# openfheorg/openfhe-development

Hardware: AMD Instinct MI355X
Metric: NTT GB/s vs HBM roofline + CKKS EvalMultKeySwitch/sec, N=2^16 L=30, 1/2/4/8 GPU (higher is better)
Workload: dtype u64; 1 GPU; batched fwd+inv negacyclic NTT, N=2^16, L=30 x 60-bit limbs, 1024 polynomials per GPU (BASELINE configs[1]); global_batch=1024, parallelism=batch-sharded x1, no data-path collective

## Files before the change

openfhe-development_amd/csrc/basis_kernels.h:

```cpp
#ifndef FHE_BASIS_KERNELS_H
#define FHE_BASIS_KERNELS_H
#include "modarith.h"
#include "launch.h"
#include "ntt_kernels.h"
#include "elemwise_kernels.h"
#include "ntt_static.h"

namespace fhe {


struct ConvTables {
    const TwPair* hatInv;
    const uint64_t* hatMod;
    const uint64_t* srcQ;
    const uint64_t* dstQ;
    const uint64_t* dstMu;
    const uint64_t* dstRed;
    const double* srcQInv;
    const uint64_t* alphaMod;
};

struct ConvArgs {
    const uint64_t* in;
    uint64_t* out;
// ... 48 lines not shown
        for (uint32_t i = 0; i < g.nSrcAll; ++i) {
            const uint64_t yi = mul_shoup(ina[(uint64_t)i << g.logN], hpa[2 * i], hpa[2 * i + 1], g.allSrcQ[i]);
            nu += (double)yi * g.allQInv[i];
        }
    }
    const uint32_t alpha = EXACT && (!CHUNK || g.last) ? (uint32_t)nu : 0u;

    for (uint32_t j = 0; j < g.nDst; ++j) {
        uint64_t h[NSRC];
#pragma unroll
        for (int i = 0; i < NSRC; ++i)
            h[i] = FHE_ULOAD64(g.tb.hatMod, (uint64_t)j * NSRC + i);
        const uint64_t p = FHE_ULOAD64(g.tb.dstQ, j);
        const uint64_t mulo = FHE_ULOAD64(g.tb.dstMu, 2 * j), muhi = FHE_ULOAD64(g.tb.dstMu, 2 * j + 1);
        if (SUM8 == 2) {
            const uint32_t k = 64u - (uint32_t)__builtin_clzll(p);
            uint64_t v       = 0;
#pragma unroll
            for (int c0 = 0; c0 < NSRC; c0 += 8) {
                if (c0 && c0 >= (int)g.nSrc)
                    break;
                sum8s s8;
                sum8s_clear(s8);
#pragma unroll
                for (int i = c0; i < c0 + 8 && i < NSRC; ++i) {
                    uint32_t y0, y1, h0, h1;
                    split30(y[i], y0, y1);
                    split30(h[i], h0, h1);
                    sum8s_add(s8, y0, y1, h0, h1);
                }
                const uint64_t rj = sum8s_reduce(s8, p, k, mulo, muhi);
                v                 = c0 ? add_mod(v, rj, p) : rj;
            }
            if (CHUNK && g.acc)
                v = add_mod(v, out[(uint64_t)j << g.logN], p);
            if (EXACT && (!CHUNK || g.last))
                v = sub_mod(v, g.tb.alphaMod[(uint64_t)alpha * g.nDst + j], p);
            out[(uint64_t)j << g.logN] = v;
            continue;
        }
        {
            static_assert(SUM8 == 1 || SUM8 == 2, "SUM8 selects one of the two column-sum forms");
            const uint32_t k = 64u - (uint32_t)__builtin_clzll(p);
            uint64_t v       = 0;
#pragma unroll
            for (int c0 = 0; c0 < NSRC; c0 += 8) {
                if (c0 && c0 >= (int)g.nSrc)
                    break;
                sum8 s8;
                sum8_clear(s8);
#pragma unroll
                for (int i = c0; i < c0 + 8 && i < NSRC; ++i)
                    sum8_add(s8, y[i], h[i]);
                const uint64_t rj = sum8_reduce(s8, p, k, mulo, muhi);
                v                 = c0 ? add_mod(v, rj, p) : rj;
            }
            if (CHUNK && g.acc)
                v = add_mod(v, out[(uint64_t)j << g.logN], p);
            if (EXACT && (!CHUNK || g.last))
                v = sub_mod(v, g.tb.alphaMod[(uint64_t)alpha * g.nDst + j], p);
            out[(uint64_t)j << g.logN] = v;
        }
    }
}

constexpr int kMaxDigits = 8;
struct KsInnerArgs {
    const uint64_t* c;
    const uint64_t* digits[kMaxDigits];
    const uint64_t* keyB;
    const uint64_t* keyA;
    uint64_t* out0;
    uint64_t* out1;
    const LimbConst* lc;
    const uint64_t* mu128;
    const uint64_t* red;
    uint32_t logN, batch, sizeQl, sizeQ, sizeP, numDigits, alpha;
    uint32_t nc[kMaxDigits];
    uint32_t j0, acc;
};
FHE_GLOBAL void FHE_LAUNCH_BOUNDS(kThreads) ks_inner_product_kernel(const KsInnerArgs g) {
    const uint32_t t          = FHE_TID;
    const uint32_t tilesPerRow = (1u << g.logN) >> kTileLog ? ((1u << g.logN) >> kTileLog) : 1u;
    const uint32_t sizeQlP    = g.sizeQl + g.sizeP;
    const uint32_t xcd = FHE_BID & 7u, slot = FHE_BID >> 3;
    const uint32_t b   = slot % g.batch;
    const uint32_t grp = (slot / g.batch) * 8u + xcd;
    const uint32_t tr = grp % tilesPerRow;
    const uint32_t i  = grp / tilesPerRow;
    if (i >= sizeQlP)
        return;
    const uint32_t idx  = i < g.sizeQl ? i : i + (g.sizeQ - g.sizeQl);
    const LimbConst lc  = g.lc[idx];
    const uint64_t mulo = g.mu128[2 * idx], muhi = g.mu128[2 * idx + 1];
    const uint64_t redc = g.red[idx];
    const uint32_t redM = (uint32_t)redc, redR = (uint32_t)(redc >> 32);
    FHE_BOUND_CHECK(redR == 255u || redR >= 3u, "key switch: the quotient estimate on a modulus below 36 bits");
    const uint32_t N    = 1u << g.logN;
    const uint32_t rEnd = ((tr + 1u) << kTileLog) < N ? ((tr + 1u) << kTileLog) : N;
    const uint64_t q = lc.q;
    for (uint32_t r = (tr << kTileLog) + t; r < rEnd; r += kThreads) {
        sum8 s0, s1;
        sum8_clear(s0);
        sum8_clear(s1);
        for (uint32_t j = 0; j < g.numDigits; ++j) {
            const uint32_t start = (g.j0 + j) * g.alpha;
            const uint32_t sz    = sizeQlP - g.nc[j];
            uint64_t d;
            if (i >= start && i < start + sz)
                d = g.c[(((uint64_t)b * g.sizeQl + i) << g.logN) + r];
            else {
                const uint32_t pos = i < start ? i : i - sz;
                d = g.digits[j][(((uint64_t)b * g.nc[j] + pos) << g.logN) + r];
            }
            if (redR != 255u)
                d -= (uint64_t)((uint32_t)(((d >> 32) * redM) >> 32) >> redR) * q;
            else {
                d = csub(d, q << 3);
                d = csub(d, q << 2);
                d = csub(d, q << 1);
            }
            d = csub(d, q);
            FHE_BOUND_CHECK(d < q, "key switch: a digit of q or more enters the 64-bit column sums");
            const uint64_t koff = (((uint64_t)(g.j0 + j) * (g.sizeQ + g.sizeP) + idx) << g.logN) + r;
            sum8_add(s0, d, g.keyB[koff]);
            sum8_add(s1, d, g.keyA[koff]);
        }
        const uint64_t ooff = (((uint64_t)b * sizeQlP + i) << g.logN) + r;
        uint64_t v0 = sum8_reduce(s0, q, lc.msb, mulo, muhi), v1 = sum8_reduce(s1, q, lc.msb, mulo, muhi);
        if (g.acc) {
            v0 = add_mod(v0, g.out0[ooff], q);
            v1 = add_mod(v1, g.out1[ooff], q);
        }
        g.out0[ooff] = v0;
        g.out1[ooff] = v1;
    }
}

constexpr int kMaxMultiKeys = 16;
struct KsInnerMultiArgs {
    const uint64_t* c;
    const uint64_t* digits[kMaxDigits];
    const uint64_t* keyB[kMaxMultiKeys];
    const uint64_t* keyA[kMaxMultiKeys];
    uint64_t* out0[kMaxMultiKeys];
    uint64_t* out1[kMaxMultiKeys];
    const uint64_t* first;
    const TwPair* firstC;
    const LimbConst* lc;
    const uint64_t* mu128;
    const uint64_t* red;
    uint32_t logN, batch, sizeQl, sizeQ, sizeP, numDigits, alpha, nKeys;
    uint32_t nc[kMaxDigits];
};
struct alignas(16) U64x2 {
    uint64_t a, b;
};
template <int CPL>
FHE_HD void ld_cpl(const uint64_t* p, uint64_t (&v)[CPL]) {
    if constexpr (CPL == 2) {
        const U64x2 w = *reinterpret_cast<const U64x2*>(p);
        v[0] = w.a, v[1] = w.b;
    }
    else
        v[0] = p[0];
}
template <int CPL>
FHE_HD void st_cpl(uint64_t* p, const uint64_t (&v)[CPL]) {
    if constexpr (CPL == 2)
        *reinterpret_cast<U64x2*>(p) = U64x2{v[0], v[1]};
    else
        p[0] = v[0];
}
template <int ND, int CPL = 1, bool PF = true>
FHE_GLOBAL void FHE_LAUNCH_BOUNDS(kThreads) ks_inner_multi_kernel(const KsInnerMultiArgs g) {
    const uint32_t t           = FHE_TID;
    const uint32_t tilesPerRow = (1u << g.logN) >> kTileLog ? ((1u << g.logN) >> kTileLog) : 1u;
    const uint32_t sizeQlP     = g.sizeQl + g.sizeP;
    const uint32_t xcd = FHE_BID & 7u, slot = FHE_BID >> 3;
    const uint32_t b   = slot % g.batch;
    const uint32_t grp = (slot / g.batch) * 8u + xcd;
    const uint32_t tr = grp % tilesPerRow;
    const uint32_t i  = grp / tilesPerRow;
    if (i >= sizeQlP)
        return;
    const uint32_t idx  = i < g.sizeQl ? i : i + (g.sizeQ - g.sizeQl);
    const LimbConst lc  = g.lc[idx];
    const uint64_t mulo = g.mu128[2 * idx], muhi = g.mu128[2 * idx + 1];
    const uint64_t redc = g.red[idx];
    const uint32_t redM = (uint32_t)redc, redR = (uint32_t)(redc >> 32);
    FHE_BOUND_CHECK(redR == 255u || redR >= 3u, "key switch: the quotient estimate on a modulus below 36 bits");
    const bool addFirst = g.first != nullptr && i < g.sizeQl;
    TwPair fc{0, 0};
    if (addFirst)
        fc = g.firstC[i];
    const uint32_t N    = 1u << g.logN;
    const uint32_t rEnd = ((tr + 1u) << kTileLog) < N ? ((tr + 1u) << kTileLog) : N;
    const uint64_t q = lc.q;
    const uint64_t ooff0 = ((uint64_t)b * sizeQlP + i) << g.logN;
    const uint64_t* src[ND];
    uint64_t koffJ[ND];
#pragma unroll
    for (int j = 0; j < ND; ++j) {
        const uint32_t jj    = (uint32_t)j < g.numDigits ? (uint32_t)j : g.numDigits - 1u;
        const uint32_t start = jj * g.alpha;
        const uint32_t sz    = sizeQlP - g.nc[jj];
        const bool own       = i >= start && i < start + sz;
        const uint32_t pos   = i < start ? i : i - sz;
        src[j] = own ? g.c + (((uint64_t)b * g.sizeQl + i) << g.logN) : g.digits[jj] + (((uint64_t)b * g.nc[jj] + pos) << g.logN);
        koffJ[j] = ((uint64_t)jj * (g.sizeQ + g.sizeP) + idx) << g.logN;
    }
    const uint64_t* firstRow = addFirst ? g.first + (((uint64_t)b * g.sizeQl + i) << g.logN) : nullptr;
    for (uint32_t r = (tr << kTileLog) + CPL * t; r < rEnd; r += CPL * kThreads) {
        uint64_t d[ND][CPL];
#pragma unroll
        for (int j = 0; j < ND; ++j)
            ld_cpl<CPL>(src[j] + r, d[j]);
        uint64_t fraw[CPL] = {};
        if (addFirst)
            ld_cpl<CPL>(firstRow + r, fraw);
        uint64_t kb[ND][CPL], ka[ND][CPL], nb[ND][CPL], na[ND][CPL];
#pragma unroll
        for (int j = 0; j < ND; ++j) {
            ld_cpl<CPL>(g.keyB[0] + koffJ[j] + r, kb[j]);
            ld_cpl<CPL>(g.keyA[0] + koffJ[j] + r, ka[j]);
        }
#pragma unroll
        for (int j = 0; j < ND; ++j)
#pragma unroll
            for (int u = 0; u < CPL; ++u) {
                uint64_t v = d[j][u];
                if (redR != 255u)
                    v -= (uint64_t)((uint32_t)(((v >> 32) * redM) >> 32) >> redR) * q;
                else {
                    v = csub(v, q << 3);
                    v = csub(v, q << 2);
                    v = csub(v, q << 1);
                }
                d[j][u] = csub(v, q);
                FHE_BOUND_CHECK(d[j][u] < q, "key switch: a digit of q or more enters the 64-bit column sums");
            }
        uint64_t f[CPL];
#pragma unroll
        for (int u = 0; u < CPL; ++u)
            f[u] = addFirst ? mul_shoup(fraw[u], fc.w, fc.wp, q) : 0;
        for (uint32_t kk = 0; kk < g.nKeys; ++kk) {
            if (PF) {
                if (kk + 1u < g.nKeys) {
                    const uint64_t* kB = g.keyB[kk + 1u];
                    const uint64_t* kA = g.keyA[kk + 1u];
#pragma unroll
                    for (int j = 0; j < ND; ++j) {
                        ld_cpl<CPL>(kB + koffJ[j] + r, nb[j]);
                        ld_cpl<CPL>(kA + koffJ[j] + r, na[j]);
                    }
                }
            }
            else if (kk) {
                const uint64_t* kB = g.keyB[kk];
                const uint64_t* kA = g.keyA[kk];
#pragma unroll
                for (int j = 0; j < ND; ++j) {
                    ld_cpl<CPL>(kB + koffJ[j] + r, kb[j]);
                    ld_cpl<CPL>(kA + koffJ[j] + r, ka[j]);
                }
            }
            uint64_t v0[CPL], v1[CPL];
#pragma unroll
            for (int u = 0; u < CPL; ++u) {
                sum8 s0, s1;
                sum8_clear(s0);
                sum8_clear(s1);
#pragma unroll
                for (int j = 0; j < ND; ++j)
                    if ((uint32_t)j < g.numDigits) {
                        sum8_add(s0, d[j][u], kb[j][u]);
                        sum8_add(s1, d[j][u], ka[j][u]);
                    }
                v0[u] = sum8_reduce(s0, q, lc.msb, mulo, muhi);
                v1[u] = sum8_reduce(s1, q, lc.msb, mulo, muhi);
                if (addFirst)
                    v0[u] = add_mod(v0[u], f[u], q);
            }
            if (PF && kk + 1u < g.nKeys) {
#pragma unroll
                for (int j = 0; j < ND; ++j)
#pragma unroll
                    for (int u = 0; u < CPL; ++u)
                        kb[j][u] = nb[j][u], ka[j][u] = na[j][u];
            }
            st_cpl<CPL>(g.out0[kk] + ooff0 + r, v0);
            st_cpl<CPL>(g.out1[kk] + ooff0 + r, v1);
        }
    }
}

struct InnerRowsArgs {
    const uint64_t* x[kMaxDigits];
    const uint64_t* k0[kMaxDigits];
    const uint64_t* k1[kMaxDigits];
    uint64_t* out0;
    uint64_t* out1;
    const LimbConst* lc;
    const uint64_t* mu128;
    uint32_t logN, batch, rows, nTerms;
    uint32_t acc;
    uint8_t keyRow[kMaxLimbs];
    LimbSel sel;
};
FHE_GLOBAL void FHE_LAUNCH_BOUNDS(kThreads) inner_rows_kernel(const InnerRowsArgs g) {
    const uint32_t t           = FHE_TID;
    const uint32_t N           = 1u << g.logN;
    const uint32_t tilesPerRow = N >> kTileLog ? (N >> kTileLog) : 1u;
    const uint32_t tr          = FHE_BID % tilesPerRow;
    const uint32_t row         = FHE_BID / tilesPerRow;
    const uint32_t i           = row % g.rows;
    const uint32_t idx         = g.sel.idx[i];
    const LimbConst lc         = g.lc[idx];
    const uint64_t mulo = g.mu128[2 * idx], muhi = g.mu128[2 * idx + 1];
    const uint64_t q    = lc.q;
    const uint32_t rEnd = ((tr + 1u) << kTileLog) < N ? ((tr + 1u) << kTileLog) : N;
    const uint64_t xoff = (uint64_t)row << g.logN;
    const uint64_t koff = (uint64_t)g.keyRow[i] << g.logN;
    const bool two      = g.k1[0] != nullptr;
    for (uint32_t r = (tr << kTileLog) + 2u * t; r < rEnd; r += 2u * kThreads) {
        sum8 a0, a1, b0, b1;
        sum8_clear(a0);
        sum8_clear(a1);
        sum8_clear(b0);
        sum8_clear(b1);
        for (uint32_t j = 0; j < g.nTerms; ++j) {
            const uint64_t x0 = g.x[j][xoff + r], x1 = g.x[j][xoff + r + 1];
            sum8_add(a0, x0, g.k0[j][koff + r]);
            sum8_add(a1, x1, g.k0[j][koff + r + 1]);
            if (two) {
                sum8_add(b0, x0, g.k1[j][koff + r]);
                sum8_add(b1, x1, g.k1[j][koff + r + 1]);
            }
        }
        uint64_t v0 = sum8_reduce(a0, q, lc.msb, mulo, muhi), v1 = sum8_reduce(a1, q, lc.msb, mulo, muhi);
        if (g.acc) {
            v0 = add_mod(v0, g.out0[xoff + r], q);
            v1 = add_mod(v1, g.out0[xoff + r + 1], q);
        }
        g.out0[xoff + r]     = v0;
        g.out0[xoff + r + 1] = v1;
        if (two) {
            v0 = sum8_reduce(b0, q, lc.msb, mulo, muhi), v1 = sum8_reduce(b1, q, lc.msb, mulo, muhi);
            if (g.acc) {
                v0 = add_mod(v0, g.out1[xoff + r], q);
                v1 = add_mod(v1, g.out1[xoff + r + 1], q);
            }
            g.out1[xoff + r]     = v0;
            g.out1[xoff + r + 1] = v1;
        }
    }
}

constexpr int kMaxBsgsIn = 16;
struct BsgsInnerArgs {
    const uint64_t* rot;
    const uint64_t* const* diag;
    uint64_t* out;
    const LimbConst* lc;
    const uint64_t* mu128;
    uint32_t logN, batch, sizeQl, sizeQ, sizeP, nIn, nInPad, j0, nOut, accumulate;
    uint32_t k[kMaxBsgsIn];
};
template <int NIN, int CPL>
FHE_GLOBAL void FHE_LAUNCH_BOUNDS(kThreads) bsgs_inner_kernel(const BsgsInnerArgs g) {
    const uint32_t t           = FHE_TID;
    const uint32_t N           = 1u << g.logN;
    const uint32_t tilesPerRow = (N >> kTileLog) ? (N >> kTileLog) : 1u;
    const uint32_t sizeQlP     = g.sizeQl + g.sizeP;
    const uint32_t nGroups     = sizeQlP * tilesPerRow, per = 2u * g.batch;
    const uint32_t xcd = FHE_BID & 7u, slot = FHE_BID >> 3;
    const uint32_t grp = (slot / per) * 8u + xcd, local = slot % per;
    if (grp >= nGroups)
        return;
    const uint32_t e = local / g.batch, b = local % g.batch;
    const uint32_t l = grp / tilesPerRow, tr = grp % tilesPerRow;
    const uint32_t idx  = l < g.sizeQl ? l : l + (g.sizeQ - g.sizeQl);
    const LimbConst lc  = g.lc[idx];
    const uint64_t mulo = g.mu128[2 * idx], muhi = g.mu128[2 * idx + 1];
    const uint64_t rotStride = ((uint64_t)2 * g.batch * sizeQlP) << g.logN;
    const uint64_t rotOff    = (((uint64_t)e * g.batch + b) * sizeQlP + l) << g.logN;
    const uint64_t outStride = ((uint64_t)g.batch * sizeQlP) << g.logN;
    const uint64_t outOff    = ((((uint64_t)e * g.nOut) * g.batch + b) * sizeQlP + l) << g.logN;
    const uint32_t rEnd      = ((tr + 1u) << kTileLog) < N ? ((tr + 1u) << kTileLog) : N;
    for (uint32_t r = (tr << kTileLog) + CPL * t; r < rEnd; r += CPL * kThreads) {
        uint64_t x[NIN][CPL], y[NIN][CPL], yn[NIN][CPL];
        uint32_t jb[CPL];
#pragma unroll
        for (int u = 0; u < CPL; ++u)
            jb[u] = bitrev32(r + (uint32_t)u, g.logN);
#pragma unroll
        for (int j = 0; j < NIN; ++j) {
            const uint32_t jj  = (uint32_t)j < g.nIn ? (uint32_t)j : g.nIn - 1u;
            const uint64_t* xp = g.rot + ((uint64_t)jj * rotStride + rotOff);
            const uint32_t kj  = g.k[jj];
#pragma unroll
            for (int u = 0; u < CPL; ++u)
                x[j][u] = xp[automorph_source(jb[u], kj, g.logN)];
        }
        const uint32_t lr = (l << g.logN) + r;
        {
            const uint64_t* const* drow = g.diag + g.j0;
#pragma unroll
            for (int j = 0; j < NIN; ++j)
                ld_cpl<CPL>(drow[j] + lr, y[j]);
        }
        for (uint32_t i = 0; i < g.nOut; ++i) {
            {
                const uint32_t in = i + 1u < g.nOut ? i + 1u : i;
                const uint64_t* const* drow = g.diag + (uint64_t)in * g.nInPad + g.j0;
#pragma unroll
                for (int j = 0; j < NIN; ++j)
                    ld_cpl<CPL>(drow[j] + lr, yn[j]);
            }
            uint64_t v[CPL] = {};
#pragma unroll
            for (int j0 = 0; j0 < NIN; j0 += 8) {
#pragma unroll
                for (int u = 0; u < CPL; ++u) {
                    sum8 s;
                    sum8_clear(s);
#pragma unroll
                    for (int j = j0; j < j0 + 8 && j < NIN; ++j)
                        sum8_add(s, x[j][u], y[j][u]);
                    const uint64_t rj = sum8_reduce(s, lc.q, lc.msb, mulo, muhi);
                    v[u]              = j0 ? add_mod(v[u], rj, lc.q) : rj;
// ... 23 lines not shown
```

openfhe-development_amd/csrc/fhe_hip.cpp:

```cpp
#include "../../include/fhe_hip.h"

#include <algorithm>
#include <cmath>
#include <cstdio>
#include <cstdlib>
#include <map>
#include <mutex>
#include <shared_mutex>
#include <string>
#include <vector>

#include "basis_kernels.h"
#include "bfv_kernels.h"
#include "elemwise_kernels.h"
#include "host_math.h"
#include "ntt_kernels.h"
#include "ntt_static.h"
#include "ntt_row8.h"
#include "rt.h"
#include "sampler_kernels.h"
#include "blake2_kernels.h"

using namespace fhe;

// ... 1804 lines not shown
        for (uint32_t i = 0; i < sizeQl; ++i)
            dst.push_back(c->q[i]);
        if (fhe_status s = conv_build(c, src, dst, &lv->down)) {
            ks_level_free(lv);
            return s;
        }
        std::vector<TwPair> pinv(sizeQl);
        for (uint32_t i = 0; i < sizeQl; ++i) {
            const uint64_t v = host::invmod(host::prod_mod(src, -1, c->q[i]), c->q[i]);
            pinv[i]          = TwPair{v, host::shoup(v, c->q[i])};
        }
        void* d       = nullptr;
        const char* e = rt::dmalloc(&d, pinv.size() * sizeof(TwPair));
        if (!e) {
            p->owned.push_back(d);
            e = rt::h2d(d, pinv.data(), pinv.size() * sizeof(TwPair), nullptr);
        }
        if (!e)
            e = rt::sync(nullptr);
        if (e) {
            ks_level_free(lv);
            return fail(FHE_ERR_DEVICE, std::string("fhe_keyswitch: building the level tables: ") + e);
        }
        lv->d_PInv = (TwPair*)d;
    }
    p->levels[sizeQl] = lv;
    *out              = lv;
    return FHE_OK;
}

extern "C" fhe_status fhe_ks_key_alloc(fhe_ks_plan* p, fhe_ks_key** out) {
    ARG_CHECK(p && out, "fhe_ks_key_alloc: null argument");
    RT_CHECK(rt::set_device(p->ctx->device));
    fhe_ks_key* k = new fhe_ks_key;
    k->plan       = p;
    k->words      = (size_t)p->numPartQ * (p->sizeQ + p->sizeP) << p->ctx->logN;
    if (rt::dmalloc((void**)&k->d_b, k->words * 8) || rt::dmalloc((void**)&k->d_a, k->words * 8)) {
        fhe_ks_key_destroy(k);
        return fail(FHE_ERR_ALLOC, "fhe_ks_key_alloc: device allocation failed");
    }
    *out = k;
    return FHE_OK;
}
extern "C" fhe_status fhe_ks_key_upload(fhe_ks_plan* p, const uint64_t* keyB, const uint64_t* keyA, fhe_ks_key** out) {
    ARG_CHECK(keyB && keyA, "fhe_ks_key_upload: null key");
    fhe_ks_key* k = nullptr;
    if (fhe_status s = fhe_ks_key_alloc(p, &k))
        return s;
    RT_CHECK(rt::h2d(k->d_b, keyB, k->words * 8, nullptr));
    RT_CHECK(rt::h2d(k->d_a, keyA, k->words * 8, nullptr));
    RT_CHECK(rt::sync(nullptr));
    *out = k;
    return FHE_OK;
}
extern "C" fhe_status fhe_ks_key_wrap(fhe_ks_plan* p, uint64_t* devB, uint64_t* devA, fhe_ks_key** out) {
    ARG_CHECK(p && devB && devA && out, "fhe_ks_key_wrap: null argument");
    fhe_ks_key* k = new fhe_ks_key;
    k->plan       = p;
    k->words      = (size_t)p->numPartQ * (p->sizeQ + p->sizeP) << p->ctx->logN;
    k->d_b        = devB;
    k->d_a        = devA;
    k->owned      = false;
    *out          = k;
    return FHE_OK;
}
extern "C" void fhe_ks_key_destroy(fhe_ks_key* k) {
    if (!k)
        return;
    if (k->owned && k->d_b)
        rt::dfree(k->d_b);
    if (k->owned && k->d_a)
        rt::dfree(k->d_a);
    delete k;
}
extern "C" uint64_t* fhe_ks_key_devptr(fhe_ks_key* k, int which) { return k ? (which ? k->d_a : k->d_b) : nullptr; }
extern "C" size_t fhe_ks_key_words(const fhe_ks_key* k) { return k ? k->words : 0; }

struct KsLayout {
    size_t coef = 0, e0 = 0, e1 = 0, md = 0, pcoef = 0, d2 = 0, k0 = 0, k1 = 0, total = 0;
    std::vector<size_t> dig;
};
static KsLayout ks_layout(const fhe_ks_plan* p, uint32_t sizeQl, uint32_t batch) {
    KsLayout w;
    const size_t N = (size_t)1 << p->ctx->logN;
    const uint32_t numParts = std::min((sizeQl + p->alpha - 1) / p->alpha, p->numPartQ);
    w.dig.assign(numParts, 0);
    size_t off = 0;
    w.coef = off, off += (size_t)batch * sizeQl * N;
    for (uint32_t j = 0; j < numParts; ++j) {
        const uint32_t start = p->alpha * j;
        const uint32_t sz    = (j == numParts - 1) ? sizeQl - start : p->alpha;
        w.dig[j] = off, off += (size_t)batch * (sizeQl - sz + p->sizeP) * N;
    }
    w.e0 = off, off += (size_t)batch * (sizeQl + p->sizeP) * N;
    w.e1 = off, off += (size_t)batch * (sizeQl + p->sizeP) * N;
    w.md = off, off += (size_t)2 * batch * sizeQl * N;
    w.pcoef = off, off += (size_t)2 * batch * p->sizeP * N;
    w.d2 = off, off += (size_t)batch * sizeQl * N;
    w.k0 = off, off += (size_t)batch * sizeQl * N;
    w.k1 = off, off += (size_t)batch * sizeQl * N;
    w.total = off;
    return w;
}
extern "C" size_t fhe_ks_workspace_bytes(const fhe_ks_plan* p, uint32_t sizeQl, uint32_t batch) {
    if (!p || sizeQl < 1 || sizeQl > p->sizeQ || batch < 1)
        return 0;
    return ks_layout(p, sizeQl, batch).total * 8;
}

static fhe_status mod_down_core(fhe_ks_plan* p, fhe_ks_plan::Level* lv, const uint64_t* x, uint32_t nTow, uint64_t* pcoef,
                                uint64_t* md, void* st, fhe_conv* down = nullptr, const NttEpilogue* epi = nullptr) {
    fhe_ctx* c            = p->ctx;
    const uint32_t sizeQl = lv->sizeQl, sizeP = p->sizeP, sizeQlP = sizeQl + sizeP;
    std::vector<uint32_t> pIdx(sizeP);
    for (uint32_t j = 0; j < sizeP; ++j)
        pIdx[j] = p->sizeQ + j;
    if (fhe_status s = ntt_run(c, true, x, pcoef, pIdx.data(), sizeP, nTow, st, sizeQlP, sizeQl))
        return s;
    if (fhe_status s = fhe_approx_switch_basis(down ? down : lv->down, pcoef, sizeP, 0, md, sizeQl, 0, nTow, st))
        return s;
    return ntt_run(c, false, md, md, nullptr, sizeQl, nTow, st, 0, 0, 0, 0, epi);
}
static fhe_status mod_down_tail(fhe_ks_plan* p, fhe_ks_plan::Level* lv, const uint64_t* x, const uint64_t* md, uint32_t nTow,
                                uint64_t* out, bool accumulate, void* st) {
    const uint32_t sizeQl = lv->sizeQl, sizeQlP = sizeQl + p->sizeP;
    if (accumulate)
        return elem_run<OP_SUB_MUL_CONST_ACC>(p->ctx, out, x, md, lv->d_PInv, nullptr, sizeQl, nTow, st, "fhe_approx_mod_down",
                                              sizeQlP, 0);
    return elem_run<OP_SUB_MUL_CONST>(p->ctx, out, x, md, lv->d_PInv, nullptr, sizeQl, nTow, st, "fhe_approx_mod_down", sizeQlP, 0);
}
static fhe_status mod_down_run(fhe_ks_plan* p, fhe_ks_plan::Level* lv, const uint64_t* x, uint32_t nTow, uint64_t* out,
                               uint64_t* pcoef, uint64_t* md, void* st) {
    if (fhe_status s = mod_down_core(p, lv, x, nTow, pcoef, md, st))
        return s;
    return mod_down_tail(p, lv, x, md, nTow, out, false, st);
}

static fhe_status ks_precompute_run(fhe_ks_plan* p, fhe_ks_plan::Level* lv, const uint64_t* cin, uint32_t batch,
                                    uint64_t* ws, const KsLayout& w, void* st) {
    fhe_ctx* c            = p->ctx;
    const uint32_t sizeQl = lv->sizeQl;
    if (fhe_status s = fhe_ntt_inv_oop(c, cin, ws + w.coef, nullptr, sizeQl, batch, st))
        return s;
    for (uint32_t j = 0; j < lv->numParts; ++j) {
        const uint32_t nc = (uint32_t)lv->cidx[j].size();
        uint64_t* dj      = ws + w.dig[j];
        if (fhe_status s = fhe_approx_switch_basis(lv->up[j], ws + w.coef, sizeQl, p->alpha * j, dj, nc, 0, batch, st))
            return s;
        if (fhe_status s = ntt_run(c, false, dj, dj, lv->cidx[j].data(), nc, batch, st, 0, 0, 0, 0, nullptr, false))
            return s;
    }
    return FHE_OK;
}
static fhe_status ks_inner_multi_launch(fhe_ks_plan* p, fhe_ks_plan::Level* lv, const fhe_ks_key* const* keys, uint32_t nKeys,
                                        const uint64_t* cin, uint32_t batch, uint64_t* const* e0, uint64_t* const* e1,
                                        const uint64_t* first, const TwPair* dP, uint64_t* ws, const KsLayout& w, void* st,
                                        uint32_t towOff = 0) {
    fhe_ctx* c            = p->ctx;
    const uint32_t sizeQl = lv->sizeQl, sizeP = p->sizeP, sizeQlP = sizeQl + sizeP;
    const uint32_t tilesPerRow = c->N >= (uint32_t)kTile ? (c->N >> kTileLog) : 1u;
    for (uint32_t t0 = 0; t0 < nKeys; t0 += (uint32_t)kMaxMultiKeys) {
        KsInnerMultiArgs g;
        const uint32_t nt = std::min<uint32_t>(kMaxMultiKeys, nKeys - t0);
        for (uint32_t j = 0; j < (uint32_t)kMaxDigits; ++j) {
            g.nc[j]     = j < lv->numParts ? (uint32_t)lv->cidx[j].size() : 0u;
            g.digits[j] = j < lv->numParts ? ws + w.dig[j] + (((size_t)towOff * g.nc[j]) << c->logN) : nullptr;
        }
        for (uint32_t t = 0; t < (uint32_t)kMaxMultiKeys; ++t) {
            const uint32_t tt = t < nt ? t0 + t : t0;
            g.keyB[t] = keys[tt]->d_b, g.keyA[t] = keys[tt]->d_a, g.out0[t] = e0[tt], g.out1[t] = e1[tt];
        }
        g.c = cin + (((size_t)towOff * sizeQl) << c->logN), g.first = first, g.firstC = dP;
        g.lc = c->d_lc, g.mu128 = c->d_mu128, g.red = c->d_red;
        g.logN = c->logN, g.batch = batch, g.sizeQl = sizeQl, g.sizeQ = p->sizeQ, g.sizeP = sizeP;
        g.numDigits = lv->numParts, g.alpha = p->alpha, g.nKeys = nt;
        const uint64_t grid = (((uint64_t)tilesPerRow * sizeQlP + 7) / 8) * 8 * batch;
        static const uint32_t ksm = env_u32("FHE_KSM", 1);
        uintptr_t bits = (uintptr_t)g.c | (uintptr_t)g.first;
        for (uint32_t j = 0; j < lv->numParts && j < (uint32_t)kMaxDigits; ++j)
            bits |= (uintptr_t)g.digits[j];
        for (uint32_t t = 0; t < nt; ++t)
            bits |= (uintptr_t)g.keyB[t] | (uintptr_t)g.keyA[t] | (uintptr_t)g.out0[t] | (uintptr_t)g.out1[t];
        const bool wide = (bits & 15u) == 0 && c->N >= 2;
        if (lv->numParts <= 3 && ksm == 1 && wide)
            FHE_LAUNCH((ks_inner_multi_kernel<3, 2, true>), grid, st, g);
        else if (lv->numParts <= 3 && ksm == 2 && wide)
            FHE_LAUNCH((ks_inner_multi_kernel<3, 2, false>), grid, st, g);
        else if (lv->numParts <= 3 && ksm == 3)
            FHE_LAUNCH((ks_inner_multi_kernel<3, 1, false>), grid, st, g);
        else if (lv->numParts <= 3)
            FHE_LAUNCH((ks_inner_multi_kernel<3>), grid, st, g);
        else if (lv->numParts <= 4)
            FHE_LAUNCH((ks_inner_multi_kernel<4>), grid, st, g);
        else
            FHE_LAUNCH((ks_inner_multi_kernel<8>), grid, st, g);
        LAUNCH_CHECK();
    }
    return FHE_OK;
}
static fhe_status ks_inner_run(fhe_ks_plan* p, fhe_ks_plan::Level* lv, const fhe_ks_key* key, const uint64_t* cin,
                               uint32_t batch, uint64_t* e0, uint64_t* e1, uint64_t* ws, const KsLayout& w, void* st,
                               uint32_t towOff = 0) {
    fhe_ctx* c            = p->ctx;
    const uint32_t sizeQl = lv->sizeQl, sizeP = p->sizeP, sizeQlP = sizeQl + sizeP;
    const uint32_t tilesPerRow = c->N >= (uint32_t)kTile ? (c->N >> kTileLog) : 1u;
    if (lv->numParts <= (uint32_t)kMaxDigits)
        return ks_inner_multi_launch(p, lv, &key, 1, cin, batch, &e0, &e1, nullptr, nullptr, ws, w, st, towOff);
    for (uint32_t j0 = 0; j0 < lv->numParts; j0 += (uint32_t)kMaxDigits) {
        KsInnerArgs g;
        const uint32_t nd = std::min<uint32_t>(kMaxDigits, lv->numParts - j0);
        for (uint32_t j = 0; j < (uint32_t)kMaxDigits; ++j) {
            g.nc[j]     = j < nd ? (uint32_t)lv->cidx[j0 + j].size() : 0u;
            g.digits[j] = j < nd ? ws + w.dig[j0 + j] + (((size_t)towOff * g.nc[j]) << c->logN) : nullptr;
        }
        g.c = cin + (((size_t)towOff * sizeQl) << c->logN), g.keyB = key->d_b, g.keyA = key->d_a;
        g.out0 = e0, g.out1 = e1;
        g.lc = c->d_lc, g.mu128 = c->d_mu128, g.red = c->d_red;
        g.logN = c->logN, g.batch = batch, g.sizeQl = sizeQl, g.sizeQ = p->sizeQ, g.sizeP = sizeP;
        g.numDigits = nd, g.alpha = p->alpha, g.j0 = j0, g.acc = j0 > 0;
        FHE_LAUNCH(ks_inner_product_kernel, (((uint64_t)tilesPerRow * sizeQlP + 7) / 8) * 8 * batch, st, g);
        LAUNCH_CHECK();
    }
    return FHE_OK;
}
static fhe_status ks_inner_multi_run(fhe_ks_plan* p, fhe_ks_plan::Level* lv, const fhe_ks_key* const* keys, uint32_t nKeys,
                                     const uint64_t* cin, uint32_t batch, uint64_t* const* e0, uint64_t* const* e1,
                                     const uint64_t* first, const TwPair* dP, uint64_t* ws, const KsLayout& w, void* st) {
    if (lv->numParts <= (uint32_t)kMaxDigits)
        return ks_inner_multi_launch(p, lv, keys, nKeys, cin, batch, e0, e1, first, dP, ws, w, st);
    const uint32_t sizeQl = lv->sizeQl, sizeQlP = sizeQl + p->sizeP;
    for (uint32_t t = 0; t < nKeys; ++t) {
        if (fhe_status s = ks_inner_run(p, lv, keys[t], cin, batch, e0[t], e1[t], ws, w, st))
            return s;
        if (first)
            if (fhe_status s = elem_run<OP_MUL_CONST_ADD>(p->ctx, e0[t], first, e0[t], dP, nullptr, sizeQl, batch, st,
                                                          "fhe_eval_fast_rotation_ext", 0, 0, sizeQlP, 0, sizeQlP, 0))
                return s;
    }
    return FHE_OK;
}
extern "C" fhe_status fhe_inner_product(fhe_ctx* c, uint32_t nTerms, const uint64_t* const* x, const uint64_t* const* k0,
                                        const uint64_t* const* k1, const uint32_t* keyRow, const uint32_t* limbIdx,
                                        uint32_t rows, uint32_t batch, uint64_t* out0, uint64_t* out1, void* st) {
    ARG_CHECK(c && x && k0 && out0, "fhe_inner_product: null argument");
    ARG_CHECK((k1 != nullptr) == (out1 != nullptr), "fhe_inner_product: the second key and the second output go together");
    ARG_CHECK(batch >= 1, "fhe_inner_product: batch must be >= 1");
    ARG_CHECK(nTerms >= 1, "fhe_inner_product: no terms");
    InnerRowsArgs g;
    if (fhe_status s = make_sel(c, limbIdx, rows, &g.sel, "fhe_inner_product"))
        return s;
    for (uint32_t i = 0; i < (uint32_t)kMaxLimbs; ++i) {
        const uint32_t kr = i < rows ? (keyRow ? keyRow[i] : i) : 0u;
        ARG_CHECK(kr < 256u, "fhe_inner_product: key row out of range");
        g.keyRow[i] = (uint8_t)kr;
    }
    for (uint32_t j = 0; j < nTerms; ++j)
        ARG_CHECK(x[j] && k0[j] && (!k1 || k1[j]), "fhe_inner_product: null term");
    RT_CHECK(rt::set_device(c->device));
    g.out0 = out0, g.out1 = out1, g.lc = c->d_lc, g.mu128 = c->d_mu128;
    g.logN = c->logN, g.batch = batch, g.rows = rows;
    const uint32_t tilesPerRow = c->N >= (uint32_t)kTile ? (c->N >> kTileLog) : 1u;
    for (uint32_t t0 = 0; t0 < nTerms; t0 += (uint32_t)kMaxDigits) {
        const uint32_t nt = std::min<uint32_t>(kMaxDigits, nTerms - t0);
        for (uint32_t j = 0; j < (uint32_t)kMaxDigits; ++j) {
            g.x[j]  = j < nt ? x[t0 + j] : nullptr;
            g.k0[j] = j < nt ? k0[t0 + j] : nullptr;
            g.k1[j] = (j < nt && k1) ? k1[t0 + j] : nullptr;
        }
        g.nTerms = nt, g.acc = t0 > 0;
        FHE_LAUNCH(inner_rows_kernel, (uint64_t)tilesPerRow * rows * batch, st, g);
        LAUNCH_CHECK();
    }
    return FHE_OK;
}
static fhe_status ks_fast_run(fhe_ks_plan* p, fhe_ks_plan::Level* lv, const fhe_ks_key* key, const uint64_t* cin,
                              uint32_t batch, uint64_t* out0, uint64_t* out1, uint64_t* ws, const KsLayout& w, void* st,
                              bool accumulate) {
    fhe_ctx* c            = p->ctx;
    const uint32_t sizeQl = lv->sizeQl;
    if (fhe_status s = ks_inner_run(p, lv, key, cin, batch, ws + w.e0, ws + w.e1, ws, w, st))
        return s;
    if (ntt_epilogue_supported(c)) {
        NttEpilogue epi;
        epi.mode = accumulate ? 2u : 1u, epi.split = batch, epi.aStride = sizeQl + p->sizeP, epi.aFirst = 0;
        epi.A = ws + w.e0, epi.C = lv->d_PInv, epi.out0 = out0, epi.out1 = out1;
        return mod_down_core(p, lv, ws + w.e0, 2 * batch, ws + w.pcoef, ws + w.md, st, nullptr, &epi);
    }
    if (fhe_status s = mod_down_core(p, lv, ws + w.e0, 2 * batch, ws + w.pcoef, ws + w.md, st))
        return s;
    if (fhe_status s = mod_down_tail(p, lv, ws + w.e0, ws + w.md, batch, out0, accumulate, st))
        return s;
    return mod_down_tail(p, lv, ws + w.e1, ws + w.md + ((size_t)batch * sizeQl << c->logN), batch, out1, accumulate, st);
}
static fhe_status keyswitch_run(fhe_ks_plan* p, const fhe_ks_key* key, const uint64_t* cin, uint32_t sizeQl,
                                uint32_t batch, uint64_t* out0, uint64_t* out1, uint64_t* ws, const KsLayout& w,
                                void* st, bool accumulate = false) {
    fhe_ks_plan::Level* lv = nullptr;
    if (fhe_status s = ks_level(p, sizeQl, &lv))
        return s;
    if (fhe_status s = ks_precompute_run(p, lv, cin, batch, ws, w, st))
        return s;
    return ks_fast_run(p, lv, key, cin, batch, out0, out1, ws, w, st, accumulate);
}

extern "C" fhe_status fhe_keyswitch_hybrid(fhe_ks_plan* p, const fhe_ks_key* key, const uint64_t* cin, uint32_t sizeQl,
                                           uint32_t batch, uint64_t* out0, uint64_t* out1, void* ws, size_t wsBytes,
                                           void* st) {
    ARG_CHECK(p && key && cin && out0 && out1 && ws, "fhe_keyswitch_hybrid: null argument");
    ARG_CHECK(key->plan == p, "fhe_keyswitch_hybrid: key belongs to another plan");
    ARG_CHECK(sizeQl >= 1 && sizeQl <= p->sizeQ && batch >= 1, "fhe_keyswitch_hybrid: bad level or batch");
    const KsLayout w = ks_layout(p, sizeQl, batch);
    ARG_CHECK(wsBytes >= w.total * 8, "fhe_keyswitch_hybrid: workspace too small");
    RT_CHECK(rt::set_device(p->ctx->device));
    return keyswitch_run(p, key, cin, sizeQl, batch, out0, out1, (uint64_t*)ws, w, st);
}

extern "C" fhe_status fhe_keyswitch_hybrid_acc(fhe_ks_plan* p, const fhe_ks_key* key, const uint64_t* cin, uint32_t sizeQl,
                                               uint32_t batch, uint64_t* acc0, uint64_t* acc1, void* ws, size_t wsBytes, void* st) {
    ARG_CHECK(p && key && cin && acc0 && acc1 && ws, "fhe_keyswitch_hybrid_acc: null argument");
    ARG_CHECK(key->plan == p, "fhe_keyswitch_hybrid_acc: key belongs to another plan");
    ARG_CHECK(sizeQl >= 1 && sizeQl <= p->sizeQ && batch >= 1, "fhe_keyswitch_hybrid_acc: bad level or batch");
    const KsLayout w = ks_layout(p, sizeQl, batch);
    ARG_CHECK(wsBytes >= w.total * 8, "fhe_keyswitch_hybrid_acc: workspace too small");
    RT_CHECK(rt::set_device(p->ctx->device));
    return keyswitch_run(p, key, cin, sizeQl, batch, acc0, acc1, (uint64_t*)ws, w, st, true);
}

extern "C" fhe_status fhe_ckks_eval_mult(fhe_ks_plan* p, const fhe_ks_key* key, const uint64_t* a0, const uint64_t* a1,
                                         const uint64_t* b0, const uint64_t* b1, uint32_t sizeQl, uint32_t batch,
                                         uint64_t* c0, uint64_t* c1, void* wsv, size_t wsBytes, void* st) {
    ARG_CHECK(p && key && a0 && a1 && b0 && b1 && c0 && c1 && wsv, "fhe_ckks_eval_mult: null argument");
    ARG_CHECK(key->plan == p, "fhe_ckks_eval_mult: key belongs to another plan");
    ARG_CHECK(sizeQl >= 1 && sizeQl <= p->sizeQ && batch >= 1, "fhe_ckks_eval_mult: bad level or batch");
    const KsLayout w = ks_layout(p, sizeQl, batch);
    ARG_CHECK(wsBytes >= w.total * 8, "fhe_ckks_eval_mult: workspace too small");
    fhe_ctx* c   = p->ctx;
    uint64_t* ws = (uint64_t*)wsv;
    RT_CHECK(rt::set_device(c->device));
    if (fhe_status s = fhe_tensor(c, a0, a1, b0, b1, c0, c1, ws + w.d2, nullptr, sizeQl, batch, st))
        return s;
    return keyswitch_run(p, key, ws + w.d2, sizeQl, batch, c0, c1, ws, w, st, true);
}

#define KS_COMMON_CHECKS(who)                                                                              \
    ARG_CHECK(p && ws, who ": null argument");                                                             \
    ARG_CHECK(sizeQl >= 1 && sizeQl <= p->sizeQ && batch >= 1, who ": bad level or batch");                \
    const KsLayout w = ks_layout(p, sizeQl, batch);                                                        \
    ARG_CHECK(wsBytes >= w.total * 8, who ": workspace too small");                                        \
    RT_CHECK(rt::set_device(p->ctx->device));                                                              \
    fhe_ks_plan::Level* lv = nullptr;                                                                      \
    if (fhe_status s_ = ks_level(p, sizeQl, &lv))                                                          \
        return s_;

extern "C" fhe_status fhe_ks_precompute(fhe_ks_plan* p, const uint64_t* c1, uint32_t sizeQl, uint32_t batch, void* ws,
                                        size_t wsBytes, void* st) {
    KS_COMMON_CHECKS("fhe_ks_precompute")
    ARG_CHECK(c1, "fhe_ks_precompute: null argument");
    return ks_precompute_run(p, lv, c1, batch, (uint64_t*)ws, w, st);
}
extern "C" fhe_status fhe_ks_fast_keyswitch(fhe_ks_plan* p, const fhe_ks_key* key, const uint64_t* c1, uint32_t sizeQl,
                                            uint32_t batch, uint64_t* out0, uint64_t* out1, void* ws, size_t wsBytes,
                                            void* st) {
    KS_COMMON_CHECKS("fhe_ks_fast_keyswitch")
    ARG_CHECK(key && c1 && out0 && out1 && key->plan == p, "fhe_ks_fast_keyswitch: bad key or null argument");
    return ks_fast_run(p, lv, key, c1, batch, out0, out1, (uint64_t*)ws, w, st, false);
}
extern "C" fhe_status fhe_eval_fast_rotation(fhe_ks_plan* p, const fhe_ks_key* key, const uint64_t* c0, const uint64_t* c1,
                                             uint32_t k, uint32_t sizeQl, uint32_t batch, uint64_t* out0, uint64_t* out1,
                                             void* ws, size_t wsBytes, void* st) {
    KS_COMMON_CHECKS("fhe_eval_fast_rotation")
    ARG_CHECK(key && c0 && c1 && out0 && out1 && key->plan == p, "fhe_eval_fast_rotation: bad key or null argument");
    ARG_CHECK(k % 2 == 1, "Automorphism index not odd");
    uint64_t* wsp = (uint64_t*)ws;
    fhe_ctx* c    = p->ctx;
    if (fhe_status s = ks_fast_run(p, lv, key, c1, batch, wsp + w.k0, wsp + w.k1, wsp, w, st, false))
        return s;
    if (fhe_status s = fhe_add(c, wsp + w.k0, wsp + w.k0, c0, nullptr, sizeQl, batch, st))
        return s;
    if (fhe_status s = fhe_automorph(c, out0, wsp + w.k0, k, 1, nullptr, sizeQl, batch, st))
        return s;
    return fhe_automorph(c, out1, wsp + w.k1, k, 1, nullptr, sizeQl, batch, st);
}
extern "C" fhe_status fhe_eval_automorphism(fhe_ks_plan* p, const fhe_ks_key* key, const uint64_t* c0, const uint64_t* c1,
                                            uint32_t k, uint32_t sizeQl, uint32_t batch, uint64_t* out0, uint64_t* out1,
                                            void* ws, size_t wsBytes, void* st) {
    if (fhe_status s = fhe_ks_precompute(p, c1, sizeQl, batch, ws, wsBytes, st))
        return s;
    return fhe_eval_fast_rotation(p, key, c0, c1, k, sizeQl, batch, out0, out1, ws, wsBytes, st);
}

static fhe_status ext_limbs(const fhe_ks_plan* p, uint32_t sizeQl, std::vector<uint32_t>& idx) {
    idx.resize(sizeQl + p->sizeP);
    for (uint32_t i = 0; i < sizeQl; ++i)
        idx[i] = i;
    for (uint32_t j = 0; j < p->sizeP; ++j)
        idx[sizeQl + j] = p->sizeQ + j;
    return FHE_OK;
}
static fhe_status ks_pmodq(fhe_ks_plan* p, fhe_ks_plan::Level* lv, TwPair** d) {
    std::lock_guard<std::mutex> lock(p->cacheMutex);
    if (!lv->d_PModq) {
        fhe_ctx* c = p->ctx;
        std::vector<uint64_t> pm(p->sizeP);
        for (uint32_t j = 0; j < p->sizeP; ++j)
            pm[j] = c->q[p->sizeQ + j];
        std::vector<TwPair> h(lv->sizeQl);
        for (uint32_t i = 0; i < lv->sizeQl; ++i) {
            const uint64_t v = host::prod_mod(pm, -1, c->q[i]);
            h[i]             = TwPair{v, host::shoup(v, c->q[i])};
        }
        void* dp = nullptr;
        RT_CHECK(rt::dmalloc(&dp, h.size() * sizeof(TwPair)));
        p->owned.push_back(dp);
        RT_CHECK(rt::h2d(dp, h.data(), h.size() * sizeof(TwPair), nullptr));
        RT_CHECK(rt::sync(nullptr));
        lv->d_PModq = (TwPair*)dp;
    }
    *d = lv->d_PModq;
    return FHE_OK;
}
extern "C" fhe_status fhe_ks_ext(fhe_ks_plan* p, const uint64_t* cin, uint32_t sizeQl, uint32_t batch, uint64_t* out, void* st) {
    ARG_CHECK(p && cin && out, "fhe_ks_ext: null argument");
    ARG_CHECK(sizeQl >= 1 && sizeQl <= p->sizeQ && batch >= 1, "fhe_ks_ext: bad level or batch");
    fhe_ctx* c = p->ctx;
    RT_CHECK(rt::set_device(c->device));
    fhe_ks_plan::Level* lv = nullptr;
    if (fhe_status s = ks_level(p, sizeQl, &lv))
        return s;
    TwPair* dP = nullptr;
    if (fhe_status s = ks_pmodq(p, lv, &dP))
        return s;
    const uint32_t sizeQlP = sizeQl + p->sizeP;
    if (fhe_status s = zero_rows(c, out, sizeQlP, sizeQl, p->sizeP, batch, st))
        return s;
    return elem_run<OP_MUL_CONST>(c, out, cin, nullptr, dP, nullptr, sizeQl, batch, st, "fhe_ks_ext", 0, 0, 0, 0, sizeQlP, 0);
}
extern "C" fhe_status fhe_ks_fast_keyswitch_ext(fhe_ks_plan* p, const fhe_ks_key* key, const uint64_t* c1, uint32_t sizeQl,
                                                uint32_t batch, uint64_t* out0, uint64_t* out1, void* ws, size_t wsBytes,
                                                void* st) {
    KS_COMMON_CHECKS("fhe_ks_fast_keyswitch_ext")
    ARG_CHECK(key && c1 && out0 && out1 && key->plan == p, "fhe_ks_fast_keyswitch_ext: bad key or null argument");
    return ks_inner_run(p, lv, key, c1, batch, out0, out1, (uint64_t*)ws, w, st);
}
extern "C" fhe_status fhe_eval_fast_rotation_ext(fhe_ks_plan* p, const fhe_ks_key* key, const uint64_t* c0, const uint64_t* c1,
                                                 uint32_t k, int addFirst, uint32_t sizeQl, uint32_t batch, uint64_t* out0,
                                                 uint64_t* out1, void* ws, size_t wsBytes, void* st) {
    KS_COMMON_CHECKS("fhe_eval_fast_rotation_ext")
    ARG_CHECK(key && c0 && c1 && out0 && out1 && key->plan == p, "fhe_eval_fast_rotation_ext: bad key or null argument");
    ARG_CHECK(k % 2 == 1, "Automorphism index not odd");
    fhe_ctx* c    = p->ctx;
    uint64_t* wsp = (uint64_t*)ws;
    const uint32_t sizeQlP = sizeQl + p->sizeP;
    if (addFirst) {
        TwPair* dP = nullptr;
        if (fhe_status s = ks_pmodq(p, lv, &dP))
            return s;
        uint64_t *e0 = wsp + w.e0, *e1 = wsp + w.e1;
        if (fhe_status s = ks_inner_multi_run(p, lv, &key, 1, c1, batch, &e0, &e1, c0, dP, wsp, w, st))
            return s;
    }
    else if (fhe_status s = ks_inner_run(p, lv, key, c1, batch, wsp + w.e0, wsp + w.e1, wsp, w, st))
        return s;
    std::vector<uint32_t> idx;
    ext_limbs(p, sizeQl, idx);
    if (fhe_status s = fhe_automorph(c, out0, wsp + w.e0, k, 1, idx.data(), sizeQlP, batch, st))
        return s;
    return fhe_automorph(c, out1, wsp + w.e1, k, 1, idx.data(), sizeQlP, batch, st);
}
extern "C" fhe_status fhe_ks_down(fhe_ks_plan* p, const uint64_t* x0, const uint64_t* x1, uint32_t sizeQl, uint32_t batch,
                                  uint64_t* out0, uint64_t* out1, void* ws, size_t wsBytes, void* st) {
    KS_COMMON_CHECKS("fhe_ks_down")
    ARG_CHECK(x0 && x1 && out0 && out1, "fhe_ks_down: null argument");
    uint64_t* wsp = (uint64_t*)ws;
    if (fhe_status s = mod_down_run(p, lv, x0, batch, out0, wsp + w.pcoef, wsp + w.md, st))
        return s;
    return mod_down_run(p, lv, x1, batch, out1, wsp + w.pcoef, wsp + w.md, st);
}

struct BsgsLayout {
    size_t ksTotal, rot, inner, d, outer, first, total;
};
static BsgsLayout bsgs_layout(const fhe_ks_plan* p, uint32_t sizeQl, uint32_t batch, uint32_t nIn, uint32_t nOut) {
    BsgsLayout b{};
    b.ksTotal        = ks_layout(p, sizeQl, batch * nOut).total;
    const size_t N   = (size_t)1 << p->ctx->logN;
    const size_t ext = (size_t)batch * (sizeQl + p->sizeP) * N, low = (size_t)batch * sizeQl * N;
    size_t off       = b.ksTotal;
    b.rot = off, off += (size_t)nIn * 2 * ext;
    b.inner = off, off += (size_t)nOut * 2 * ext;
    b.d = off, off += (size_t)nOut * 2 * low;
    b.outer = off, off += 2 * ext;
// ... 1528 lines not shown
```

Measured before the change: 2340 GB/s.

## Fuse CKKS tensor product terms into key-switch inner product for EvalMult

Adds a tensor-term variant of the key-switch inner-product kernel that also accumulates a0*b0 and a0*b1+a1*b0, scaled by P mod q, into the same column sums. The EvalMult path then computes only a1*b1 separately and lets mod-down produce the final c0/c1 with its epilogue. This removes the separate full tensor kernel and the later accumulate pass over c0/c1, trading them for extra loads in the inner kernel and a non-prefetch kernel variant. The fused path is enabled by default through an environment flag.

```diff
diff --git a/openfhe-development_amd/csrc/basis_kernels.h b/openfhe-development_amd/csrc/basis_kernels.h
--- a/openfhe-development_amd/csrc/basis_kernels.h
+++ b/openfhe-development_amd/csrc/basis_kernels.h
@@ -224,6 +224,8 @@
     const uint64_t* red;
     uint32_t logN, batch, sizeQl, sizeQ, sizeP, numDigits, alpha, nKeys;
     uint32_t nc[kMaxDigits];
+    const uint64_t *ta0, *ta1, *tb0, *tb1;
+    const TwPair* tenC;
 };
 struct alignas(16) U64x2 {
     uint64_t a, b;
@@ -244,8 +246,9 @@
     else
         p[0] = v[0];
 }
-template <int ND, int CPL = 1, bool PF = true>
+template <int ND, int CPL = 1, bool PF = true, bool TEN = false>
 FHE_GLOBAL void FHE_LAUNCH_BOUNDS(kThreads) ks_inner_multi_kernel(const KsInnerMultiArgs g) {
+    static_assert(!TEN || ND + 2 <= kMaxDigits, "tensor terms: two more products per sum than digits, at most 8 in all");
     const uint32_t t           = FHE_TID;
     const uint32_t tilesPerRow = (1u << g.logN) >> kTileLog ? ((1u << g.logN) >> kTileLog) : 1u;
     const uint32_t sizeQlP     = g.sizeQl + g.sizeP;
@@ -283,6 +286,14 @@
         koffJ[j] = ((uint64_t)jj * (g.sizeQ + g.sizeP) + idx) << g.logN;
     }
     const uint64_t* firstRow = addFirst ? g.first + (((uint64_t)b * g.sizeQl + i) << g.logN) : nullptr;
+    const bool ten           = TEN && i < g.sizeQl;
+    TwPair tc{0, 0};
+    uint64_t tenOff = 0;
+    if (ten) {
+        FHE_BOUND_CHECK(g.numDigits + 2u <= (uint32_t)kMaxDigits, "key switch: digits + tensor terms exceed the 8 products of a column sum");
+        tc     = g.tenC[i];
+        tenOff = ((uint64_t)b * g.sizeQl + i) << g.logN;
+    }
     for (uint32_t r = (tr << kTileLog) + CPL * t; r < rEnd; r += CPL * kThreads) {
         uint64_t d[ND][CPL];
 #pragma unroll
@@ -291,6 +302,13 @@
         uint64_t fraw[CPL] = {};
         if (addFirst)
             ld_cpl<CPL>(firstRow + r, fraw);
+        uint64_t xa0[CPL] = {}, xa1[CPL] = {}, xb0[CPL] = {}, xb1[CPL] = {};
+        if (ten) {
+            ld_cpl<CPL>(g.ta0 + tenOff + r, xa0);
+            ld_cpl<CPL>(g.ta1 + tenOff + r, xa1);
+            ld_cpl<CPL>(g.tb0 + tenOff + r, xb0);
+            ld_cpl<CPL>(g.tb1 + tenOff + r, xb1);
+        }
         uint64_t kb[ND][CPL], ka[ND][CPL], nb[ND][CPL], na[ND][CPL];
 #pragma unroll
         for (int j = 0; j < ND; ++j) {
@@ -316,6 +334,14 @@
 #pragma unroll
         for (int u = 0; u < CPL; ++u)
             f[u] = addFirst ? mul_shoup(fraw[u], fc.w, fc.wp, q) : 0;
+        if (ten) {
+#pragma unroll
+            for (int u = 0; u < CPL; ++u) {
+                FHE_BOUND_CHECK(xa0[u] < q && xa1[u] < q && xb0[u] < q && xb1[u] < q, "key switch: a tensor operand of q or more enters the 64-bit column sums");
+                xa0[u] = mul_shoup(xa0[u], tc.w, tc.wp, q);
+                xa1[u] = mul_shoup(xa1[u], tc.w, tc.wp, q);
+            }
+        }
         for (uint32_t kk = 0; kk < g.nKeys; ++kk) {
             if (PF) {
                 if (kk + 1u < g.nKeys) {
@@ -349,6 +375,11 @@
                         sum8_add(s0, d[j][u], kb[j][u]);
                         sum8_add(s1, d[j][u], ka[j][u]);
                     }
+                if (ten) {
+                    sum8_add(s0, xa0[u], xb0[u]);
+                    sum8_add(s1, xa0[u], xb1[u]);
+                    sum8_add(s1, xa1[u], xb0[u]);
+                }
                 v0[u] = sum8_reduce(s0, q, lc.msb, mulo, muhi);
                 v1[u] = sum8_reduce(s1, q, lc.msb, mulo, muhi);
                 if (addFirst)
diff --git a/openfhe-development_amd/csrc/fhe_hip.cpp b/openfhe-development_amd/csrc/fhe_hip.cpp
--- a/openfhe-development_amd/csrc/fhe_hip.cpp
+++ b/openfhe-development_amd/csrc/fhe_hip.cpp
@@ -1980,10 +1980,14 @@
     }
     return FHE_OK;
 }
+struct KsTensorOps {
+    const uint64_t *a0, *a1, *b0, *b1;
+    const TwPair* dP;
+};
 static fhe_status ks_inner_multi_launch(fhe_ks_plan* p, fhe_ks_plan::Level* lv, const fhe_ks_key* const* keys, uint32_t nKeys,
                                         const uint64_t* cin, uint32_t batch, uint64_t* const* e0, uint64_t* const* e1,
                                         const uint64_t* first, const TwPair* dP, uint64_t* ws, const KsLayout& w, void* st,
-                                        uint32_t towOff = 0) {
+                                        uint32_t towOff = 0, const KsTensorOps* ten = nullptr) {
     fhe_ctx* c            = p->ctx;
     const uint32_t sizeQl = lv->sizeQl, sizeP = p->sizeP, sizeQlP = sizeQl + sizeP;
     const uint32_t tilesPerRow = c->N >= (uint32_t)kTile ? (c->N >> kTileLog) : 1u;
@@ -2002,6 +2006,9 @@
         g.lc = c->d_lc, g.mu128 = c->d_mu128, g.red = c->d_red;
         g.logN = c->logN, g.batch = batch, g.sizeQl = sizeQl, g.sizeQ = p->sizeQ, g.sizeP = sizeP;
         g.numDigits = lv->numParts, g.alpha = p->alpha, g.nKeys = nt;
+        g.ta0 = g.ta1 = g.tb0 = g.tb1 = nullptr, g.tenC = nullptr;
+        if (ten)
+            g.ta0 = ten->a0, g.ta1 = ten->a1, g.tb0 = ten->b0, g.tb1 = ten->b1, g.tenC = ten->dP;
         const uint64_t grid = (((uint64_t)tilesPerRow * sizeQlP + 7) / 8) * 8 * batch;
         static const uint32_t ksm = env_u32("FHE_KSM", 1);
         uintptr_t bits = (uintptr_t)g.c | (uintptr_t)g.first;
@@ -2009,8 +2016,18 @@
             bits |= (uintptr_t)g.digits[j];
         for (uint32_t t = 0; t < nt; ++t)
             bits |= (uintptr_t)g.keyB[t] | (uintptr_t)g.keyA[t] | (uintptr_t)g.out0[t] | (uintptr_t)g.out1[t];
+        if (ten)
+            bits |= (uintptr_t)g.ta0 | (uintptr_t)g.ta1 | (uintptr_t)g.tb0 | (uintptr_t)g.tb1;
         const bool wide = (bits & 15u) == 0 && c->N >= 2;
-        if (lv->numParts <= 3 && ksm == 1 && wide)
+        if (ten) {
+            if (nKeys != 1 || towOff != 0 || first || !wide || lv->numParts > 6)
+                return fail(FHE_ERR_UNSUPPORTED, "key switch: no inner-product instance with tensor terms for this shape");
+            if (lv->numParts <= 3)
+                FHE_LAUNCH((ks_inner_multi_kernel<3, 2, false, true>), grid, st, g);
+            else
+                FHE_LAUNCH((ks_inner_multi_kernel<6, 2, false, true>), grid, st, g);
+        }
+        else if (lv->numParts <= 3 && ksm == 1 && wide)
             FHE_LAUNCH((ks_inner_multi_kernel<3, 2, true>), grid, st, g);
         else if (lv->numParts <= 3 && ksm == 2 && wide)
             FHE_LAUNCH((ks_inner_multi_kernel<3, 2, false>), grid, st, g);
@@ -2154,6 +2171,7 @@
     return keyswitch_run(p, key, cin, sizeQl, batch, acc0, acc1, (uint64_t*)ws, w, st, true);
 }
 
+static fhe_status ks_pmodq(fhe_ks_plan* p, fhe_ks_plan::Level* lv, TwPair** d);
 extern "C" fhe_status fhe_ckks_eval_mult(fhe_ks_plan* p, const fhe_ks_key* key, const uint64_t* a0, const uint64_t* a1,
                                          const uint64_t* b0, const uint64_t* b1, uint32_t sizeQl, uint32_t batch,
                                          uint64_t* c0, uint64_t* c1, void* wsv, size_t wsBytes, void* st) {
@@ -2165,6 +2183,30 @@
     fhe_ctx* c   = p->ctx;
     uint64_t* ws = (uint64_t*)wsv;
     RT_CHECK(rt::set_device(c->device));
+    static const uint32_t fuse = env_u32("FHE_EVALMULT_FUSE", 1);
+    fhe_ks_plan::Level* lv = nullptr;
+    if (fhe_status s = ks_level(p, sizeQl, &lv))
+        return s;
+    const uintptr_t bits = (uintptr_t)ws | (uintptr_t)key->d_b | (uintptr_t)key->d_a | (uintptr_t)a0 | (uintptr_t)a1 | (uintptr_t)b0 | (uintptr_t)b1;
+    if (fuse >= 1 && lv->numParts <= 6 && ntt_epilogue_supported(c) && (bits & 15u) == 0 && c->N >= 2) {
+        KsTensorOps ten{a0, a1, b0, b1, nullptr};
+        TwPair* dP = nullptr;
+        if (fhe_status s = ks_pmodq(p, lv, &dP))
+            return s;
+        ten.dP = dP;
+        if (fhe_status s = elem_run<OP_MUL>(c, ws + w.d2, a1, b1, nullptr, nullptr, sizeQl, batch, st, "fhe_ckks_eval_mult"))
+            return s;
+        if (fhe_status s = ks_precompute_run(p, lv, ws + w.d2, batch, ws, w, st))
+            return s;
+        uint64_t *e0 = ws + w.e0, *e1 = ws + w.e1;
+        const fhe_ks_key* keys[1] = {key};
+        if (fhe_status s = ks_inner_multi_launch(p, lv, keys, 1, ws + w.d2, batch, &e0, &e1, nullptr, nullptr, ws, w, st, 0, &ten))
+            return s;
+        NttEpilogue epi;
+        epi.mode = 1u, epi.split = batch, epi.aStride = sizeQl + p->sizeP, epi.aFirst = 0;
+        epi.A = ws + w.e0, epi.C = lv->d_PInv, epi.out0 = c0, epi.out1 = c1;
+        return mod_down_core(p, lv, ws + w.e0, 2 * batch, ws + w.pcoef, ws + w.md, st, nullptr, &epi);
+    }
     if (fhe_status s = fhe_tensor(c, a0, a1, b0, b1, c0, c1, ws + w.d2, nullptr, sizeQl, batch, st))
         return s;
     return keyswitch_run(p, key, ws + w.d2, sizeQl, batch, c0, c1, ws, w, st, true);
```

Result: no change. 2342 GB/s, median of 2 (+0.1%).
